# Gadersd/stable-diffusion-burn

Hardware: NVIDIA H100
Metric: images_per_sec_512x512_20steps (higher is better)
Workload: dtype fp16 tensor-core operands (3-term split-fp16 on the two high-res UNet levels), fp32 accumulate

## Files before the change

### stable_diffusion_burn_b200/csrc/api.cu

```cuda
#include "../../include/sdb200.h"

#include <dlfcn.h>

#include <cstdlib>
#include <cstring>
#include <mutex>

#include "attention.cuh"
#include "kernels.cuh"
#include "model.cuh"
#include "runtime.cuh"

using namespace sdb;

struct sdb_ctx {
  Ctx c;
};

static thread_local std::string g_err;

#define API_BEGIN(ctxp)                      \
  if (!(ctxp)) {                             \
    g_err = "null context";                  \
    return 1;                                \
// ... 474 lines not shown
    c.opt_splitk_chunk = value < 1 ? 1 : value;
  else if (k == "attn_split")
    c.opt_attn_split = value;
  else if (k == "attn_regsplit")
    g_attn_regsplit = value;
  else if (k == "emb_hoist")
    c.opt_emb_hoist = value;
  else if (k == "prefetch_w")
    c.opt_prefetch_w = value;
  else if (k == "mlp_passes")
    c.opt_mlp_passes = value;
  else if (k == "gn_epilogue")
    c.opt_gn_epilogue = value;
  else if (k == "skip_merge")
    c.opt_skip_merge = value;
  else if (k == "gn_apply_ctas")
    g_gn_apply_ctas = value < 1 ? 1 : value;
  else if (k == "gn_min_pix")
    g_gn_min_pix = value < 1 ? 1 : value;
  else
    throw Error("unknown option: " + k);
  model_invalidate_graphs(c);
  API_END
}

int sdb_profile_enable(sdb_ctx* ctx, int on) {
  API_BEGIN(ctx)
  profile_collect(c);
  c.profiling = on != 0;
  API_END
// ... 406 lines not shown
```

### stable_diffusion_burn_b200/csrc/gemm_tc.cu

```cuda
#include "gemm_tc.cuh"

#include <cstring>

namespace sdb {

static constexpr int BM = 128;
static constexpr int BK = 64;
static constexpr int A_TILE_BYTES = BM * BK * 2;

template <int BN, int PASSES>
struct StageLayout {
  static constexpr int B_TILE_BYTES = BN * BK * 2;
  static constexpr int A_TILES = PASSES >= 2 ? 2 : 1;
  static constexpr int B_TILES = PASSES >= 3 ? 2 : 1;
  static constexpr int BYTES = A_TILES * A_TILE_BYTES + B_TILES * B_TILE_BYTES;
};
template <int BN>
struct AccLayout {
  static constexpr int PITCH = (BN + 4) * 4;
  static constexpr int BYTES = BM * PITCH;
  static constexpr int GN_BYTES = 32 * 1024;
};
static constexpr int EW = 8;

__device__ __noinline__ void epilogue_store(float4 f, unsigned int o32, unsigned int o16, float* out_f32, __half* out_f16,
                                            __half* out_f16_lo, int act) {
  if (act == 1) {
    f.x = __fdividef(f.x, 1.0f + __expf(-1.702f * f.x)), f.y = __fdividef(f.y, 1.0f + __expf(-1.702f * f.y));
    f.z = __fdividef(f.z, 1.0f + __expf(-1.702f * f.z)), f.w = __fdividef(f.w, 1.0f + __expf(-1.702f * f.w));
  }
  if (out_f32) *reinterpret_cast<float4*>(out_f32 + o32) = f;
  if (out_f16) {
    __half2 h[2] = {f2h2_sat(f.x, f.y), f2h2_sat(f.z, f.w)};
    *reinterpret_cast<uint2*>(out_f16 + o16) = *reinterpret_cast<uint2*>(h);
    if (out_f16_lo) {
      const float2 f0 = __half22float2(h[0]), f1 = __half22float2(h[1]);
      __half2 l[2] = {__floats2half2_rn(f.x - f0.x, f.y - f0.y), __floats2half2_rn(f.z - f1.x, f.w - f1.y)};
      *reinterpret_cast<uint2*>(out_f16_lo + o16) = *reinterpret_cast<uint2*>(l);
    }
  }
}

struct GnTile {
  int tn, img0, tile, nimg;
};
__device__ __forceinline__ GnTile gn_tile_of(const GemmParams& p, int n0, int th, int tw) {
  GnTile g;
  if (p.gn_rpi) {
    g.nimg = p.gn_nimg;
    if (p.gn_rpi >= BM)
      g.tn = 1, g.img0 = (tw * BM) / p.gn_rpi, g.tile = ((tw * BM) % p.gn_rpi) / BM;
    else
      g.tn = BM / p.gn_rpi, g.img0 = tw * g.tn, g.tile = 0;
  } else {
    g.tn = p.TN, g.img0 = n0, g.tile = th * p.tiles_w + tw, g.nimg = p.nimg;
  }
  return g;
}
__device__ __forceinline__ void gn_write_partials(const GemmParams& p, const float2* cs, int BN, int te, int nthreads, const GnTile g,
                                                  int col0, int z) {
// ... 8 lines not shown
      const float2* src = cs + q * BN + b * p.gn_bucket;
      for (int c = 0; c < p.gn_bucket; ++c) sm += src[c].x, sq += src[c].y;
    }
    if (qpi >= 2) sm += __shfl_xor_sync(0xffffffffu, sm, 1), sq += __shfl_xor_sync(0xffffffffu, sq, 1);
    if (qpi == 4) sm += __shfl_xor_sync(0xffffffffu, sm, 2), sq += __shfl_xor_sync(0xffffffffu, sq, 2);
    const int k = q / qpi, img = g.img0 + k, c0 = b * p.gn_bucket;
    if (b < nbk_tile && (q % qpi) == 0 && img < g.nimg && col0 + c0 < p.N) {
      float2* dst = reinterpret_cast<float2*>(p.gn_part) + ((size_t)img * p.gn_cap + slot) * nbk_total + (col0 + c0) / p.gn_bucket;
      *dst = make_float2(sm, sq);
    }
  }
}

enum : int { EPI_PLAIN = 0, EPI_GN = 1, EPI_LNS = 2, EPI_LNC = 3, EPI_GEGLU = 4, EPI_GEGLU_LNC = 5 };

template <int BN, int PASSES, int STAGES>
__host__ __device__ constexpr int region_bytes() {
  return STAGES * StageLayout<BN, PASSES>::BYTES > AccLayout<BN>::BYTES + AccLayout<BN>::GN_BYTES
             ? STAGES * StageLayout<BN, PASSES>::BYTES
             : AccLayout<BN>::BYTES + AccLayout<BN>::GN_BYTES;
}

template <int BN, int PASSES, int STAGES, int EPI>
__global__ void __launch_bounds__(128 + 32 * EW, 1)
gemm_tc_kernel(const __grid_constant__ GemmMaps maps, const GemmParams p) {
  constexpr bool kGN = EPI == EPI_GN, kLNS = EPI == EPI_LNS, kLNC = EPI == EPI_LNC || EPI == EPI_GEGLU_LNC;
  constexpr bool kGEGLU = EPI == EPI_GEGLU || EPI == EPI_GEGLU_LNC;
  using L = StageLayout<BN, PASSES>;
  constexpr int EG = EW / 4;
  constexpr int CSTEP = 32 * EG;
  extern __shared__ __align__(1024) uint8_t smem_raw[];
  uint8_t* smem = smem_raw + ((1024u - (smem_u32(smem_raw) & 1023u)) & 1023u);
  uint64_t* full_bar = reinterpret_cast<uint64_t*>(smem + region_bytes<BN, PASSES, STAGES>());
  uint64_t* empty_bar = full_bar + STAGES;

  const int warp = threadIdx.x >> 5;
  const int lane = threadIdx.x & 31;
  long long* const dbg = (p.dbg && blockIdx.x == 0 && blockIdx.y == 0 && blockIdx.z == 0) ? p.dbg : nullptr;
  if (dbg && threadIdx.x == 0) dbg[0] = clock64();
  if (!p.pdl_late) pdl_trigger();

  int mt = blockIdx.x;
  const int tw = mt % p.tiles_w;
  mt /= p.tiles_w;
  const int th = mt % p.tiles_h;
  const int tn = mt / p.tiles_h;
  const int w0 = tw * p.TW, h0 = th * p.TH, n0 = tn * p.TN;
  const int col0 = blockIdx.y * BN;
// ... 69 lines not shown
      for (int it = it_begin + npre; it < it_end; ++it) {
        mbar_wait(&empty_bar[s], ph ^ 1);
        mbar_expect_tx(&full_bar[s], L::BYTES);
        load_a(it, s);
        load_b(it, s);
        if (++s == STAGES) {
          s = 0;
          ph ^= 1;
        }
      }
    }
  } else if (warp >= 4) {
    pdl_wait();
    const int wg = (warp - 4) >> 2;
    {
      float acc[BN / 2];
#pragma unroll
      for (int i = 0; i < BN / 2; ++i) acc[i] = 0.f;
      int s = 0, prev = -1;
      uint32_t ph = 0;
      for (int it = it_begin; it < it_end; ++it) {
        mbar_wait(&full_bar[s], ph);
        if (dbg && threadIdx.x == 128 && it == it_begin) dbg[3] = clock64();
        const uint32_t a_hi = smem_u32(smem + s * L::BYTES) + wg * (64 * 128);
        const uint32_t a_lo = a_hi + A_TILE_BYTES;
        const uint32_t b_hi = smem_u32(smem + s * L::BYTES) + L::A_TILES * A_TILE_BYTES;
        const uint32_t b_lo = b_hi + L::B_TILE_BYTES;
        wgmma_fence();
#pragma unroll
        for (int k = 0; k < BK / 16; ++k) {
          const uint32_t koff = k * 32;
          const uint64_t da = make_sdesc_sw128(a_hi + koff);
          const uint64_t db = make_sdesc_sw128(b_hi + koff);
          Wgmma<BN>::template ss<0>(acc, da, db, 1);
          if (PASSES >= 2) Wgmma<BN>::template ss<0>(acc, make_sdesc_sw128(a_lo + koff), db, 1);
          if (PASSES >= 3) Wgmma<BN>::template ss<0>(acc, da, make_sdesc_sw128(b_lo + koff), 1);
        }
        wgmma_commit();
        wgmma_wait<1>();
        if (prev >= 0 && lane == 0) mbar_arrive(&empty_bar[prev]);
        prev = s;
        if (++s == STAGES) {
          s = 0;
          ph ^= 1;
        }
      }
      wgmma_wait<0>();
      reg_fence(acc);
      if (dbg && threadIdx.x == 128) dbg[4] = clock64();
      asm volatile("bar.sync 1, %0;" ::"n"(EW * 32) : "memory");
      float* img = reinterpret_cast<float*>(smem);
      const int r0 = wg * 64 + (warp & 3) * 16 + (lane >> 2);
#pragma unroll
      for (int j = 0; j < BN / 2; j += 2) {
        const int row = r0 + 8 * ((j >> 1) & 1), col = 8 * (j >> 2) + 2 * (lane & 3);
        *reinterpret_cast<float2*>(img + row * (AccLayout<BN>::PITCH / 4) + col) = make_float2(acc[j], acc[j + 1]);
      }
      asm volatile("bar.sync 1, %0;" ::"n"(EW * 32) : "memory");
    }
    const int q = warp & 3;
    const int half = (warp - 4) >> 2;
    const int r = q * 32 + lane;
    const int pw = w0 + r % p.TW;
    const int phh = h0 + (r / p.TW) % p.TH;
    const int pn = n0 + r / (p.TW * p.TH);
    const int row_ok = ((pw < p.W) && (phh < p.H) && (pn < p.nimg)) ? 1 : 0;
    const int m = row_ok ? ((pn * p.OH + phh * p.os + p.oa + up_a) * p.OW + pw * p.os + p.ob + up_b) : -1;

    const int sub = lane >> 3;
    const int cq = (lane & 7) * 4;
    constexpr int NCHUNK = (BN + CSTEP - 1) / CSTEP;
    int mr8[8], ao[8];
    float4 bvs[NCHUNK], ad[8];
    const float* ad_ptr = p.residual ? p.residual : p.rowbias;
    const bool res_pair = p.res_hi != nullptr;
    const bool plain = p.split_k == 1 && !kGEGLU;
    float ln_mu = 0.f, ln_rs = 0.f;
    float mu8[8], rs8[8];
    float4 us[NCHUNK];
    if constexpr (kLNC) {
      if (m >= 0) {
        const float2* sp = reinterpret_cast<const float2*>(p.ln_in) + (size_t)m * p.ln_in_slots;
        float sm = 0.f, sq = 0.f;
        for (int i = 0; i < p.ln_in_slots; ++i) {
          const float2 v = sp[i];
          sm += v.x, sq += v.y;
        }
        const float inv = 1.0f / (float)p.ln_C;
        ln_mu = sm * inv;
        ln_rs = rsqrtf(fmaxf(sq * inv - ln_mu * ln_mu, 0.f) + p.ln_eps);
      }
    }
    {
      const bool use_res = p.residual != nullptr;
#pragma unroll
      for (int i = 0; i < 8; ++i) {
        const int rr = i * 4 + sub;
        const int mr = __shfl_sync(0xffffffffu, m, rr);
        const int pnr = __shfl_sync(0xffffffffu, pn, rr);
        mr8[i] = mr;
        ao[i] = res_pair ? mr * p.ldc16 : (use_res ? mr * p.ldc : pnr * p.N);
        ad[i] = make_float4(0.f, 0.f, 0.f, 0.f);
        if constexpr (kLNC) mu8[i] = __shfl_sync(0xffffffffu, ln_mu, rr), rs8[i] = __shfl_sync(0xffffffffu, ln_rs, rr);
      }
      if constexpr (kLNC) {
#pragma unroll
        for (int j = 0; j < NCHUNK; ++j) {
          const int col = col0 + half * 32 + j * CSTEP + cq;
          us[j] = make_float4(0.f, 0.f, 0.f, 0.f);
          if (half * 32 + j * CSTEP < BN && col < p.N) us[j] = *reinterpret_cast<const float4*>(p.ln_u + col);
        }
      }
#pragma unroll
      for (int j = 0; j < NCHUNK; ++j) {
        const int col = col0 + half * 32 + j * CSTEP + cq;
        bvs[j] = make_float4(0.f, 0.f, 0.f, 0.f);
        if (plain && p.bias && half * 32 + j * CSTEP < BN && col < p.N) bvs[j] = *reinterpret_cast<const float4*>(p.bias + col);
      }
    }
    auto issue_addends = [&](int col) {
      if constexpr (kLNC) return;
      if (col >= p.N) return;
      if (res_pair) {
#pragma unroll
        for (int i = 0; i < 8; ++i)
          if (mr8[i] >= 0) {
            const uint2 h = *reinterpret_cast<const uint2*>(p.res_hi + (unsigned)(ao[i] + col));
            const uint2 l = *reinterpret_cast<const uint2*>(p.res_lo + (unsigned)(ao[i] + col));
            const float2 h0 = __half22float2(*reinterpret_cast<const __half2*>(&h.x)), h1 = __half22float2(*reinterpret_cast<const __half2*>(&h.y));
            const float2 l0 = __half22float2(*reinterpret_cast<const __half2*>(&l.x)), l1 = __half22float2(*reinterpret_cast<const __half2*>(&l.y));
            ad[i] = make_float4(h0.x + l0.x, h0.y + l0.y, h1.x + l1.x, h1.y + l1.y);
          }
        return;
      }
      if (ad_ptr == nullptr) return;
#pragma unroll
      for (int i = 0; i < 8; ++i)
        if (mr8[i] >= 0) ad[i] = *reinterpret_cast<const float4*>(ad_ptr + (unsigned)(ao[i] + col));
    };
    const bool pre_issued = plain;
    if (pre_issued) issue_addends(col0 + half * 32 + cq);

    if (p.pdl_late) pdl_trigger();
    if (dbg && threadIdx.x == 128) dbg[5] = clock64();
    constexpr uint32_t TROW = AccLayout<BN>::PITCH;
    const uint32_t arow = smem_u32(smem) + q * 32 * TROW;
    auto unstage = [&](uint32_t t, int rr) {
      float4 f;
      asm volatile("ld.shared.v4.f32 {%0, %1, %2, %3}, [%4];"
                   : "=f"(f.x), "=f"(f.y), "=f"(f.z), "=f"(f.w)
                   : "r"(t + rr * TROW + cq * 4)
                   : "memory");
      return f;
    };
    float2* const gn_cs = reinterpret_cast<float2*>(smem + AccLayout<BN>::BYTES);
    const GnTile gnt = gn_tile_of(p, n0, th, tw);
    auto store_out = [&](float4 f, int mr, int col) {
      epilogue_store(f, (unsigned)(mr * p.ldc + col), (unsigned)(mr * p.ldc16 + col), p.out_f32, p.out_f16, p.out_f16_lo, p.act);
    };

    if (!kGEGLU && p.split_k > 1) {
      const size_t Mtot = (size_t)p.nimg * p.OH * p.OW;
      float* wsbase = p.ws + (size_t)kz * Mtot * p.N;
#pragma unroll 1
      for (int c = half * 32; c < BN; c += CSTEP) {
        const int col = col0 + c + cq;
#pragma unroll
        for (int i = 0; i < 8; ++i) {
          const int rr = i * 4 + sub;
          const int mr = __shfl_sync(0xffffffffu, m, rr);
          if (mr >= 0 && col < p.N) __stcg(reinterpret_cast<float4*>(wsbase + (size_t)mr * p.N + col), unstage(arow + c * 4, rr));
        }
      }
      __threadfence();
      asm volatile("bar.sync 1, %0;" ::"n"(EW * 32) : "memory");
      unsigned int* tk = p.tickets + 2 * ((size_t)blockIdx.y * gridDim.x + blockIdx.x);
// ... 3 lines not shown
        while (atomicAdd(tk, 0u) < (unsigned)p.split_k) {
          __nanosleep(32);
          if (clock64() - t0 > 4000000000ll) __trap();
        }
        __threadfence();
      }
      asm volatile("bar.sync 1, %0;" ::"n"(EW * 32) : "memory");
      {
        const int rows_per = (BM + p.split_k - 1) / p.split_k;
        const int r0 = kz * rows_per, r1 = min(BM, r0 + rows_per);
        constexpr int C4 = BN / 4;
        constexpr int RL = (EW * 32) / C4;
        const int te = threadIdx.x - 128;
        const int rlane = te / C4, cg4 = te - rlane * C4;
        const int rpi = BM / gnt.tn;
        float4* const gn_red = reinterpret_cast<float4*>(smem + AccLayout<BN>::BYTES);
#pragma unroll 1
        for (int k = 0; k < gnt.tn; ++k) {
        float4 gsum = make_float4(0.f, 0.f, 0.f, 0.f), gsq = gsum;
        const int row_a = max(r0, k * rpi), row_b = min(r1, (k + 1) * rpi);
#pragma unroll 1
        for (int rl = row_a + rlane; rlane < RL && rl < row_b; rl += RL) {
          const int col = col0 + cg4 * 4;
          const int qw = w0 + rl % p.TW, qh = h0 + (rl / p.TW) % p.TH, qn = n0 + rl / (p.TW * p.TH);
          if (qw < p.W && qh < p.H && qn < p.nimg && col < p.N) {
            const int mr = (qn * p.OH + qh * p.os + p.oa) * p.OW + qw * p.os + p.ob;
            float4 bv = make_float4(0.f, 0.f, 0.f, 0.f), rb = bv, rs = bv;
            if (p.bias) bv = *reinterpret_cast<const float4*>(p.bias + col);
            if (p.rowbias) rb = *reinterpret_cast<const float4*>(p.rowbias + (size_t)qn * p.N + col);
            if (p.residual) rs = *reinterpret_cast<const float4*>(p.residual + (size_t)mr * p.ldc + col);
            if (p.res_hi) {
// ... 88 lines not shown
              tx.x = rrs * (tx.x - rmu * ux.x), tx.y = rrs * (tx.y - rmu * ux.y), tx.z = rrs * (tx.z - rmu * ux.z), tx.w = rrs * (tx.w - rmu * ux.w);
              tg.x = rrs * (tg.x - rmu * ug.x), tg.y = rrs * (tg.y - rmu * ug.y), tg.z = rrs * (tg.z - rmu * ug.z), tg.w = rrs * (tg.w - rmu * ug.w);
            }
            float4 y;
            y.x = (tx.x + bx.x) * gelu_erf_fast(tg.x + bg.x);
            y.y = (tx.y + bx.y) * gelu_erf_fast(tg.y + bg.y);
            y.z = (tx.z + bx.z) * gelu_erf_fast(tg.z + bg.z);
            y.w = (tx.w + bx.w) * gelu_erf_fast(tg.w + bg.w);
            epilogue_store(y, 0u, (unsigned)(mr * p.ldc16 + ocol0 + c + cq), nullptr, p.out_f16, p.out_f16_lo, 0);
          }
        }
      }
    } else {
      constexpr int NCH = NCHUNK;
      if (!pre_issued) issue_addends(col0 + half * 32 + cq);
      float lrs[8], lrq[8];
#pragma unroll
      for (int k = 0; k < 8; ++k) lrs[k] = 0.f, lrq[k] = 0.f;
      (void)lrs, (void)lrq;
#pragma unroll
      for (int j = 0; j < NCH; ++j) {
        const int c = half * 32 + j * CSTEP;
        if (c < BN) {
          const int col = col0 + c + cq;
          float4 gsum = make_float4(0.f, 0.f, 0.f, 0.f), gsq = gsum;
          (void)gsum, (void)gsq;
          if (col < p.N) {
            const uint32_t tl = arow + c * 4 + sub * TROW + cq * 4;
#pragma unroll
            for (int b4 = 0; b4 < 2; ++b4) {
              float4 t[4];
#pragma unroll
              for (int i = 0; i < 4; ++i)
                asm volatile("ld.shared.v4.f32 {%0, %1, %2, %3}, [%4];"
                             : "=f"(t[i].x), "=f"(t[i].y), "=f"(t[i].z), "=f"(t[i].w)
                             : "r"(tl + (b4 * 4 + i) * 4 * TROW)
                             : "memory");
#pragma unroll
              for (int i = 0; i < 4; ++i) {
                const int k = b4 * 4 + i;
                if (mr8[k] < 0) continue;
                float4 f = t[i];
                if constexpr (kLNC) {
                  f.x = rs8[k] * (f.x - mu8[k] * us[j].x), f.y = rs8[k] * (f.y - mu8[k] * us[j].y);
                  f.z = rs8[k] * (f.z - mu8[k] * us[j].z), f.w = rs8[k] * (f.w - mu8[k] * us[j].w);
// ... 22 lines not shown
              gsum.z += __shfl_xor_sync(0xffffffffu, gsum.z, o), gsum.w += __shfl_xor_sync(0xffffffffu, gsum.w, o);
              gsq.x += __shfl_xor_sync(0xffffffffu, gsq.x, o), gsq.y += __shfl_xor_sync(0xffffffffu, gsq.y, o);
              gsq.z += __shfl_xor_sync(0xffffffffu, gsq.z, o), gsq.w += __shfl_xor_sync(0xffffffffu, gsq.w, o);
            }
            if (sub == 0) {
              float2* d = gn_cs + q * BN + c + cq;
              d[0] = make_float2(gsum.x, gsq.x), d[1] = make_float2(gsum.y, gsq.y);
              d[2] = make_float2(gsum.z, gsq.z), d[3] = make_float2(gsum.w, gsq.w);
            }
          }
          if (j + 1 < NCH && c + CSTEP < BN) issue_addends(col0 + c + CSTEP + cq);
        }
      }
      if constexpr (kLNS) {
#pragma unroll
        for (int k = 0; k < 8; ++k) {
#pragma unroll
          for (int o = 1; o <= 4; o <<= 1) {
            lrs[k] += __shfl_xor_sync(0xffffffffu, lrs[k], o);
            lrq[k] += __shfl_xor_sync(0xffffffffu, lrq[k], o);
          }
        }
        if ((lane & 7) == 0) {
          const int slot = blockIdx.y * 2 + half;
#pragma unroll
          for (int k = 0; k < 8; ++k)
            if (mr8[k] >= 0) {
              float2* d = reinterpret_cast<float2*>(p.ln_out) + (size_t)mr8[k] * p.ln_slots + slot;
              d[0] = make_float2(lrs[k], lrq[k]);
              if (EG == 1) d[1] = make_float2(0.f, 0.f);
            }
        }
      }
      if constexpr (kGN) {
        asm volatile("bar.sync 1, %0;" ::"n"(EW * 32) : "memory");
        gn_write_partials(p, gn_cs, BN, threadIdx.x - 128, EW * 32, gnt, col0, p.up2 ? (int)blockIdx.z * p.gn_phase_slots : 0);
      }
    }
    if (dbg && threadIdx.x == 128) dbg[6] = clock64();
  }
  __syncthreads();
  if (dbg && threadIdx.x == 0) dbg[7] = clock64();
}

static constexpr int SMEM_OPTIN_MAX = 227 * 1024;
template <int BN, int PASSES>
constexpr int pick_stages() {
  constexpr int per = StageLayout<BN, PASSES>::BYTES;
  constexpr int n = (SMEM_OPTIN_MAX - 1024) / (per + 2 * 8);
  return n > 8 ? 8 : n;
}

template <int BN, int PASSES, int STAGES, int EPI>
static void launch_epi(const GemmMaps& maps, const GemmParams& p, cudaStream_t stream) {
  constexpr int smem = region_bytes<BN, PASSES, STAGES>() + 2 * STAGES * 8 + 1024;
  static_assert(smem <= SMEM_OPTIN_MAX, "shared memory per block");
  static_assert(4 * BN * 8 <= AccLayout<BN>::GN_BYTES && 2 * (EW * 32) * 4 * 16 <= AccLayout<BN>::GN_BYTES,
                "GroupNorm column sums must fit in the scratch after the accumulator image");
  static DeviceOnce once;
  if (once.first())
    SDB_CUDA(cudaFuncSetAttribute(gemm_tc_kernel<BN, PASSES, STAGES, EPI>, cudaFuncAttributeMaxDynamicSharedMemorySize, smem));
  dim3 grid(p.tiles_n * p.tiles_h * p.tiles_w, (p.N + BN - 1) / BN, p.up2 ? 4 : p.split_k);
  launch_k(gemm_tc_kernel<BN, PASSES, STAGES, EPI>, grid, dim3(128 + 32 * EW), (size_t)smem, stream, maps, p);
}
template <int BN, int PASSES, int STAGES>
static void launch_inst(const GemmMaps& maps, const GemmParams& p, cudaStream_t stream) {
  SDB_CHECK((p.gn_part != nullptr) + (p.ln_out != nullptr) + (p.ln_in != nullptr) <= 1, "one statistics role per launch");
  if constexpr (BN == 128) {
    if (p.geglu) {
      SDB_CHECK(!p.gn_part && !p.ln_out && p.split_k == 1, "GEGLU epilogue: no statistics output, no split-K");
      return p.ln_in ? launch_epi<BN, PASSES, STAGES, EPI_GEGLU_LNC>(maps, p, stream)
                     : launch_epi<BN, PASSES, STAGES, EPI_GEGLU>(maps, p, stream);
    }
  }
  SDB_CHECK(!p.geglu, "the GEGLU epilogue is built for 128-wide tiles");
  if constexpr (BN >= 128) {
    if (p.gn_part) return launch_epi<BN, PASSES, STAGES, EPI_GN>(maps, p, stream);
  }
  if constexpr (BN == 160) {
    if (p.ln_out) return launch_epi<BN, PASSES, STAGES, EPI_LNS>(maps, p, stream);
  }
  if constexpr (BN == 128 || BN == 160) {
    if (p.ln_in) return launch_epi<BN, PASSES, STAGES, EPI_LNC>(maps, p, stream);
  }
  SDB_CHECK(!p.gn_part && !p.ln_out && !p.ln_in, "this statistics epilogue is not built for this tile width");
  launch_epi<BN, PASSES, STAGES, EPI_PLAIN>(maps, p, stream);
}
bool gemm_tc_supports(int BN, int epi) {
  return epi == EPI_PLAIN || (epi == EPI_GN && BN >= 128) || (epi == EPI_LNS && BN == 160) || (epi == EPI_LNC && (BN == 128 || BN == 160));
}

template <int BN, int PASSES>
static void launch_bn(const GemmMaps& maps, const GemmParams& p, cudaStream_t stream) {
  launch_inst<BN, PASSES, pick_stages<BN, PASSES>()>(maps, p, stream);
}

void gemm_tc_launch(const GemmMaps& maps, const GemmParams& p, int BN, int passes, cudaStream_t stream) {
  SDB_CHECK(p.TN * p.TH * p.TW == BM, "M tile must cover 128 rows");
  SDB_CHECK(p.N % 32 == 0, "N must be a multiple of 32");
#define SDB_DISPATCH(bn)                                             \
  case bn:                                                           \
    if (passes == 1) launch_bn<bn, 1>(maps, p, stream);              \
    else if (passes == 2) launch_bn<bn, 2>(maps, p, stream);         \
    else launch_bn<bn, 3>(maps, p, stream);                          \
    break;
  switch (BN) {
    SDB_DISPATCH(64)
    SDB_DISPATCH(128)
    SDB_DISPATCH(160)
    SDB_DISPATCH(256)
    default:
      throw Error("unsupported BN");
  }
#undef SDB_DISPATCH
}

}
```

### stable_diffusion_burn_b200/csrc/gemm_tc.cuh

```cuda
#pragma once
#include "common.cuh"

namespace sdb {

struct GemmMaps {
  CUtensorMap a[4][2];
  CUtensorMap bx[2];
  CUtensorMap b[2];
};

struct GemmParams {
  int nimg, H, W;
  int TN, TH, TW;
  int tiles_n, tiles_h, tiles_w;
  int N;
  int kc;
  int kc0;
  int num_taps;
  int xkc, xkc0;
  int8_t tap_dh[9], tap_dw[9], tap_ph[9];
  int split_k;
  int up2, gn_phase_slots;
  float* out_f32;
  __half* out_f16;
// ... 16 lines not shown
  const float* ln_in;
  int ln_in_slots, ln_C;
  float ln_eps;
  const float* ln_u;
  const __half* res_hi;
  const __half* res_lo;
  float* ws;
  unsigned int* tickets;
  int OH, OW, os, oa, ob;
};

struct GemmLaunch {
  int BN, passes, stages;
};

void gemm_tc_launch(const GemmMaps& maps, const GemmParams& p, int BN, int passes, cudaStream_t stream);
bool gemm_tc_supports(int BN, int epi);
int gemm_tc_smem_bytes(int BN, int passes, int stages);

}
```

### stable_diffusion_burn_b200/csrc/runtime.cu

```cuda
#include "runtime.cuh"

#include <algorithm>

#include <cudaTypedefs.h>

#include <cmath>
#include <cstdlib>
#include <cstring>

namespace sdb {

int g_pdl_late = 1;
bool g_pdl_enabled = true;
int g_num_sms = 132;

void Arena::init(size_t bytes) {
  SDB_CUDA(cudaMalloc(&base, bytes));
  cap = bytes;
  off = 0;
}
void Arena::destroy() {
  if (base) cudaFree(base);
  base = nullptr;
  cap = off = 0;
// ... 193 lines not shown
    for (int jj = 0; jj < 4; ++jj)
      fprintf(stderr, "  j=%d softmax warpgroup 0: s_issued %lld s_ready %lld softmax_done %lld pv_issued %lld pv_done %lld\n",
              8 + jj, rel(jj * 8 + 0), rel(jj * 8 + 1), rel(jj * 8 + 2), rel(jj * 8 + 3), rel(jj * 8 + 4));
  }
}

static int pow2_floor(int x) {
  int p = 1;
  while (p * 2 <= x) p *= 2;
  return p;
}
static int pow2_ceil(int x) {
  int p = 1;
  while (p < x) p *= 2;
  return p;
}

void run_gemm(Ctx& c, int kind, const ActOp& a0in, const ActOp* a1in, const WeightOp& w, int passes, const Epilogue& ep,
              const ExtraK* xk) {
  ActOp a0 = a0in, a1;
  if (a1in) a1 = *a1in;
  int gn_rpi = ep.gn_rpi, gn_nimg = 0;
  const int kind_in = kind;
  if (kind == G_CONV1) {
    gn_rpi = a0.H * a0.W;
    a0.W = a0.n * a0.H * a0.W, a0.H = 1, a0.n = 1;
    if (a1in) a1.W = a1.n * a1.H * a1.W, a1.H = 1, a1.n = 1;
    kind = G_LINEAR;
  }
  SDB_CHECK(a0.C % 64 == 0, "A channels must be a multiple of 64");
// ... 47 lines not shown
    default:
      throw Error("bad gemm kind");
  }
  SDB_CHECK(w.K == p.num_taps * Ctot, "weight K does not match the operand");
  if (xk) {
    const int xC = xk->x0.C + (xk->has_x1 ? xk->x1.C : 0);
    SDB_CHECK(kind == G_CONV3 || kind == G_LINEAR, "extra-K operands need an unshifted output grid");
    SDB_CHECK(xk->x0.n == a0.n && xk->x0.H == a0.H && xk->x0.W == a0.W && xk->x0.P == 1 && xk->x0.C % 64 == 0, "extra-K geometry");
    SDB_CHECK(!xk->has_x1 || (xk->x1.n == a0.n && xk->x1.H == a0.H && xk->x1.W == a0.W && xk->x1.C % 64 == 0), "extra-K geometry");
    SDB_CHECK(xk->w.N == w.N && xk->w.K == xC, "extra-K weights");
    SDB_CHECK(passes < 2 || (xk->x0.p.lo && (!xk->has_x1 || xk->x1.p.lo)), "multi-pass GEMM needs the lo half of the extra operands");
    SDB_CHECK(passes < 3 || xk->w.p.lo, "3-pass GEMM needs the lo half of the extra weights");
    p.xkc0 = xk->x0.C / 64, p.xkc = xC / 64;
  }

  p.TW = std::min(pow2_floor(a0.W), 128);
  p.TH = std::min(128 / p.TW, pow2_ceil(a0.H));
  p.TN = 128 / (p.TW * p.TH);
  p.tiles_w = (a0.W + p.TW - 1) / p.TW;
  p.tiles_h = (a0.H + p.TH - 1) / p.TH;
  p.tiles_n = (a0.n + p.TN - 1) / p.TN;
  const int m_tiles = p.tiles_w * p.tiles_h * p.tiles_n;

  int BN;
  if (ep.geglu)
    BN = 128;
  else if (w.N % 160 == 0)
    BN = 160;
  else if (w.N % 256 == 0 && (long long)m_tiles * (w.N / 256) >= 2 * g_num_sms)
    BN = 256;
  else if (w.N % 128 == 0)
    BN = 128;
  else
    BN = 64;
  if (ep.ln_out) {
    SDB_CHECK(w.N % 160 == 0 && !ep.geglu, "LayerNorm statistics need an output width that tiles by 160");
    BN = 160;
// ... 4 lines not shown

  const int iters = p.num_taps * p.kc + p.xkc;
  int split = 1;
  if (c.opt_splitk && kind != G_CONV3_UP2 && !ep.geglu && !ep.ln_out && !ep.ln_in) {
    const int ctas = m_tiles * n_tiles;
    if (ctas <= g_num_sms / 2 && iters >= c.opt_splitk_min_iters) {
      split = std::min(std::min(g_num_sms / ctas, iters / c.opt_splitk_chunk), 16);
      if (split < 1) split = 1;
    }
  }
  if (split > 1) {
    const int per = (iters + split - 1) / split;
    split = (iters + per - 1) / per;
  }
  p.split_k = split;
  static const bool gemm_dbg = getenv("SDB_GEMM_DBG") != nullptr || getenv("SDB_LABEL_LOG") != nullptr;
  if (c.debug_sync || c.profiling || gemm_dbg) {
    char buf[256];
    snprintf(buf, sizeof(buf), "gemm kind=%d n=%d H=%d W=%d P=%d C0=%d C1=%d N=%d K=%d xk=%d BN=%d split=%d passes=%d geglu=%d epi=%s%s tile=%dx%dx%d",
             kind, a0.n, a0.H, a0.W, a0.P, a0.C, a1in ? a1.C : 0, w.N, w.K, p.xkc * 64, BN, split, passes, ep.geglu,
             ep.gn ? "gn" : (ep.ln_out ? "lns" : (ep.ln_in ? "lnc" : "-")), ep.residual16.hi ? "+r16" : (ep.residual ? "+r32" : ""), p.TN, p.TH, p.TW);
    c.dbg_label = buf;
  }

  GnPart* gn = ep.gn;
  if (gn) {
    int slots = m_tiles / p.tiles_n * split * phases_out;
    bool geom = p.TN <= 4;
    if (kind == G_LINEAR && gn_rpi > 0) {
      const long long rows = (long long)a0.W;
// ... 22 lines not shown
  p.ln_u = passes >= 3 ? ep.ln_u_full : ep.ln_u_hi;
  SDB_CHECK(!ep.ln_in || (p.ln_u && ep.ln_in_slots > 0 && ep.ln_C == w.K && kind == G_LINEAR), "LayerNorm-consuming GEMM: arguments");
  SDB_CHECK(!ep.ln_in || (!ep.residual && !ep.rowbias && !ep.residual16.hi), "LayerNorm-consuming GEMM: no residual / row bias");
  SDB_CHECK(!ep.ln_out || kind == G_LINEAR, "LayerNorm statistics: rows must be tokens");
  p.res_hi = ep.residual16.hi, p.res_lo = ep.residual16.lo;
  SDB_CHECK(!ep.residual16.hi || (ep.residual16.lo && !ep.residual && !ep.rowbias), "fp16-pair residual: needs both halves, excludes the fp32 residual / row bias");
  p.out_f32 = ep.out_f32;
  p.out_f16 = ep.out_f16.hi;
  p.out_f16_lo = ep.out_f16.lo;
  p.bias = ep.bias;
  p.rowbias = ep.rowbias;
  p.residual = ep.residual;
  p.geglu = ep.geglu;
  p.act = ep.act;
  p.pdl_late = g_pdl_late;
  p.prefetch_w = (g_pdl_enabled && c.opt_prefetch_w && m_tiles <= 4) ? 1 : 0;
  const int nout = ep.geglu ? w.N / 2 : w.N;
  p.ldc = ep.ldc ? ep.ldc : nout;
  p.ldc16 = ep.ldc16 ? ep.ldc16 : nout;
  SDB_CHECK(!(ep.rowbias && ep.residual), "epilogue takes a time-embedding row or a residual, not both");
  p.os = (kind == G_CONV3_UP2) ? 2 : 1;
  p.OH = a0.H * p.os, p.OW = a0.W * p.os;
  SDB_CHECK((double)a0.n * p.OH * p.OW * (double)std::max(p.ldc, p.ldc16) < 2147483648.0,
            "GEMM output exceeds 2^31 elements (the epilogue uses 32-bit element offsets)");

  GemmMaps maps;
  memset(&maps, 0, sizeof(maps));
  maps.a[0][0] = make_act_map(a0.p.hi, a0.C, a0.W, a0.H, a0.P, a0.n, p.TW, p.TH, p.TN);
  maps.a[0][1] = maps.a[0][0];
  if (passes >= 2) maps.a[0][1] = make_act_map(a0.p.lo, a0.C, a0.W, a0.H, a0.P, a0.n, p.TW, p.TH, p.TN);
  maps.a[1][0] = maps.a[0][0];
// ... 50 lines not shown
      SDB_CHECK((long long)m_tiles * n_tiles * split <= g_num_sms, "split-K CTAs must be co-resident");
      p.tickets = c.splitk_tickets;
    }
    {
      static const bool dbg_on = getenv("SDB_GEMM_DBG") != nullptr;
      static long long* dbg_buf = nullptr;
      if (dbg_on) {
        if (!dbg_buf) SDB_CUDA(cudaMallocManaged(&dbg_buf, 16 * sizeof(long long)));
        SDB_CUDA(cudaStreamSynchronize(c.stream));
        memset(dbg_buf, 0, 16 * sizeof(long long));
        p.dbg = dbg_buf;
      }
      const std::string label = c.dbg_label;
      {
        KernelScope ks(c, KC_GEMM, flops * phases_out, bytes * phases_out, flops * passes * phases_out);
        gemm_tc_launch(maps, p, BN, passes, c.stream);
      }
      if (dbg_on) {
        SDB_CUDA(cudaStreamSynchronize(c.stream));
        fprintf(stderr, "gemm_dbg %s | cycles since entry: prologue %lld tma0 %lld landed %lld lastmma %lld accum %lld epi %lld exit %lld | chunk0: ld %lld stage %lld finish %lld (bias %lld loads0 %lld batch0 %lld)\n",
                label.c_str(), dbg_buf[1] - dbg_buf[0], dbg_buf[2] - dbg_buf[0], dbg_buf[3] - dbg_buf[0],
                dbg_buf[4] - dbg_buf[0], dbg_buf[5] - dbg_buf[0], dbg_buf[6] - dbg_buf[0], dbg_buf[7] - dbg_buf[0], dbg_buf[9] - dbg_buf[8], dbg_buf[10] - dbg_buf[9],
                dbg_buf[11] - dbg_buf[10], dbg_buf[12] - dbg_buf[10], dbg_buf[13] - dbg_buf[12], dbg_buf[14] - dbg_buf[13]);
      }
    }
  }
}

}
```

### stable_diffusion_burn_b200/csrc/runtime.cuh

```cuda
#pragma once
#include <string>
#include <unordered_map>
#include <unordered_set>
#include <vector>

#include "common.cuh"
#include "attention.cuh"
#include "gemm_tc.cuh"
#include "kernels.cuh"

namespace sdb {

struct Arena {
  char* base = nullptr;
  size_t cap = 0, off = 0, high = 0;
  void init(size_t bytes);
  void destroy();
  void* alloc(size_t bytes);
  template <class T>
  T* get(size_t count) {
    return reinterpret_cast<T*>(alloc(count * sizeof(T)));
  }
  void reset() { off = 0; }
};
// ... 91 lines not shown
  bool finalized = false;
  std::vector<MetaCheck> meta;
  std::unordered_set<std::string> group_norms;
  std::unordered_map<std::string, float> norm_eps;
  int opt_precision = 0;
  int opt_graphs = 1;
  int opt_splitk = 1;
  int opt_splitk_min_iters = 32, opt_splitk_chunk = 8;
  int opt_skip_merge = 1;
  int opt_raw16 = 1;
  int opt_mlp_passes = 0;
  int opt_attn_split = 1;
  int opt_emb_hoist = 1;
  int opt_prefetch_w = 0;
  int opt_gn_epilogue = 1;
  int sampler_kind = 0;
  double sampler_eta = 0.0;
  uint64_t sampler_noise_seed = 0;
  bool profiling = false;
  std::vector<ProfEvent> prof;
  int64_t launches = 0;
  double cls_ms[KC_COUNT] = {0}, cls_flops[KC_COUNT] = {0}, cls_bytes[KC_COUNT] = {0};
  double cls_issued[KC_COUNT] = {0};
  int64_t cls_launches[KC_COUNT] = {0};
  struct IoBuf {
    void* p = nullptr;
    size_t cap = 0;
  } iobuf[12];
  void* io(int slot, size_t bytes);
  void io_destroy();
// ... 62 lines not shown
```

Baseline: 4.972.

## Add 64-row M tiles for linear GEMMs chosen by a wave-cost model

Templates the wgmma GEMM kernel on BM so linear layers can use 64-row M tiles. In that mode the two consumer warpgroups split the N dimension instead of M, and the epilogue handles fewer rows per warp. A simple wave-quantization cost model picks 64 or 128 rows per linear GEMM when split-K is off and the epilogue is plain or LayerNorm. This is meant to cut tail-wave waste on small-M linears (text encoder, low-res attention projections). In exchange, more CTAs each reuse operands less, and the model's fixed-cost constant is a guess.

```diff
diff --git a/stable_diffusion_burn_b200/csrc/api.cu b/stable_diffusion_burn_b200/csrc/api.cu
--- a/stable_diffusion_burn_b200/csrc/api.cu
+++ b/stable_diffusion_burn_b200/csrc/api.cu
@@ -512,6 +512,10 @@
     c.opt_gn_epilogue = value;
   else if (k == "skip_merge")
     c.opt_skip_merge = value;
+  else if (k == "linear_bm") {
+    SDB_CHECK(value == 0 || value == 64 || value == 128, "linear_bm: 0 (tile plan), 64 or 128");
+    c.opt_linear_bm = value;
+  }
   else if (k == "gn_apply_ctas")
     g_gn_apply_ctas = value < 1 ? 1 : value;
   else if (k == "gn_min_pix")
diff --git a/stable_diffusion_burn_b200/csrc/gemm_tc.cu b/stable_diffusion_burn_b200/csrc/gemm_tc.cu
--- a/stable_diffusion_burn_b200/csrc/gemm_tc.cu
+++ b/stable_diffusion_burn_b200/csrc/gemm_tc.cu
@@ -4,18 +4,17 @@
 
 namespace sdb {
 
-static constexpr int BM = 128;
 static constexpr int BK = 64;
-static constexpr int A_TILE_BYTES = BM * BK * 2;
-
-template <int BN, int PASSES>
+
+template <int BM, int BN, int PASSES>
 struct StageLayout {
+  static constexpr int A_TILE_BYTES = BM * BK * 2;
   static constexpr int B_TILE_BYTES = BN * BK * 2;
   static constexpr int A_TILES = PASSES >= 2 ? 2 : 1;
   static constexpr int B_TILES = PASSES >= 3 ? 2 : 1;
   static constexpr int BYTES = A_TILES * A_TILE_BYTES + B_TILES * B_TILE_BYTES;
 };
-template <int BN>
+template <int BM, int BN>
 struct AccLayout {
   static constexpr int PITCH = (BN + 4) * 4;
   static constexpr int BYTES = BM * PITCH;
@@ -44,6 +43,7 @@
 struct GnTile {
   int tn, img0, tile, nimg;
 };
+template <int BM>
 __device__ __forceinline__ GnTile gn_tile_of(const GemmParams& p, int n0, int th, int tw) {
   GnTile g;
   if (p.gn_rpi) {
@@ -82,24 +82,29 @@
 
 enum : int { EPI_PLAIN = 0, EPI_GN = 1, EPI_LNS = 2, EPI_LNC = 3, EPI_GEGLU = 4, EPI_GEGLU_LNC = 5 };
 
-template <int BN, int PASSES, int STAGES>
+template <int BM, int BN, int PASSES, int STAGES>
 __host__ __device__ constexpr int region_bytes() {
-  return STAGES * StageLayout<BN, PASSES>::BYTES > AccLayout<BN>::BYTES + AccLayout<BN>::GN_BYTES
-             ? STAGES * StageLayout<BN, PASSES>::BYTES
-             : AccLayout<BN>::BYTES + AccLayout<BN>::GN_BYTES;
-}
-
-template <int BN, int PASSES, int STAGES, int EPI>
+  return STAGES * StageLayout<BM, BN, PASSES>::BYTES > AccLayout<BM, BN>::BYTES + AccLayout<BM, BN>::GN_BYTES
+             ? STAGES * StageLayout<BM, BN, PASSES>::BYTES
+             : AccLayout<BM, BN>::BYTES + AccLayout<BM, BN>::GN_BYTES;
+}
+
+template <int BM, int BN, int PASSES, int STAGES, int EPI>
 __global__ void __launch_bounds__(128 + 32 * EW, 1)
 gemm_tc_kernel(const __grid_constant__ GemmMaps maps, const GemmParams p) {
   constexpr bool kGN = EPI == EPI_GN, kLNS = EPI == EPI_LNS, kLNC = EPI == EPI_LNC || EPI == EPI_GEGLU_LNC;
   constexpr bool kGEGLU = EPI == EPI_GEGLU || EPI == EPI_GEGLU_LNC;
-  using L = StageLayout<BN, PASSES>;
+  static_assert(BM == 128 || (BM == 64 && !kGN && !kGEGLU && BN % 16 == 0), "64-row tiles: plain / LayerNorm epilogues");
+  using L = StageLayout<BM, BN, PASSES>;
+  constexpr int A_TILE_BYTES = L::A_TILE_BYTES;
+  constexpr int WN = BM == 128 ? BN : BN / 2;
+  constexpr int RW = BM / 4;
+  constexpr int NR = RW / 4;
   constexpr int EG = EW / 4;
   constexpr int CSTEP = 32 * EG;
   extern __shared__ __align__(1024) uint8_t smem_raw[];
   uint8_t* smem = smem_raw + ((1024u - (smem_u32(smem_raw) & 1023u)) & 1023u);
-  uint64_t* full_bar = reinterpret_cast<uint64_t*>(smem + region_bytes<BN, PASSES, STAGES>());
+  uint64_t* full_bar = reinterpret_cast<uint64_t*>(smem + region_bytes<BM, BN, PASSES, STAGES>());
   uint64_t* empty_bar = full_bar + STAGES;
 
   const int warp = threadIdx.x >> 5;
@@ -199,17 +204,17 @@
     pdl_wait();
     const int wg = (warp - 4) >> 2;
     {
-      float acc[BN / 2];
-#pragma unroll
-      for (int i = 0; i < BN / 2; ++i) acc[i] = 0.f;
+      float acc[WN / 2];
+#pragma unroll
+      for (int i = 0; i < WN / 2; ++i) acc[i] = 0.f;
       int s = 0, prev = -1;
       uint32_t ph = 0;
       for (int it = it_begin; it < it_end; ++it) {
         mbar_wait(&full_bar[s], ph);
         if (dbg && threadIdx.x == 128 && it == it_begin) dbg[3] = clock64();
-        const uint32_t a_hi = smem_u32(smem + s * L::BYTES) + wg * (64 * 128);
+        const uint32_t a_hi = smem_u32(smem + s * L::BYTES) + (BM == 128 ? wg * (64 * 128) : 0);
         const uint32_t a_lo = a_hi + A_TILE_BYTES;
-        const uint32_t b_hi = smem_u32(smem + s * L::BYTES) + L::A_TILES * A_TILE_BYTES;
+        const uint32_t b_hi = smem_u32(smem + s * L::BYTES) + L::A_TILES * A_TILE_BYTES + (BM == 128 ? 0 : wg * (WN * 128));
         const uint32_t b_lo = b_hi + L::B_TILE_BYTES;
         wgmma_fence();
 #pragma unroll
@@ -217,9 +222,9 @@
           const uint32_t koff = k * 32;
           const uint64_t da = make_sdesc_sw128(a_hi + koff);
           const uint64_t db = make_sdesc_sw128(b_hi + koff);
-          Wgmma<BN>::template ss<0>(acc, da, db, 1);
-          if (PASSES >= 2) Wgmma<BN>::template ss<0>(acc, make_sdesc_sw128(a_lo + koff), db, 1);
-          if (PASSES >= 3) Wgmma<BN>::template ss<0>(acc, da, make_sdesc_sw128(b_lo + koff), 1);
+          Wgmma<WN>::template ss<0>(acc, da, db, 1);
+          if (PASSES >= 2) Wgmma<WN>::template ss<0>(acc, make_sdesc_sw128(a_lo + koff), db, 1);
+          if (PASSES >= 3) Wgmma<WN>::template ss<0>(acc, da, make_sdesc_sw128(b_lo + koff), 1);
         }
         wgmma_commit();
         wgmma_wait<1>();
@@ -235,33 +240,34 @@
       if (dbg && threadIdx.x == 128) dbg[4] = clock64();
       asm volatile("bar.sync 1, %0;" ::"n"(EW * 32) : "memory");
       float* img = reinterpret_cast<float*>(smem);
-      const int r0 = wg * 64 + (warp & 3) * 16 + (lane >> 2);
-#pragma unroll
-      for (int j = 0; j < BN / 2; j += 2) {
-        const int row = r0 + 8 * ((j >> 1) & 1), col = 8 * (j >> 2) + 2 * (lane & 3);
-        *reinterpret_cast<float2*>(img + row * (AccLayout<BN>::PITCH / 4) + col) = make_float2(acc[j], acc[j + 1]);
+      const int r0 = (BM == 128 ? wg * 64 : 0) + (warp & 3) * 16 + (lane >> 2);
+      const int c0 = BM == 128 ? 0 : wg * WN;
+#pragma unroll
+      for (int j = 0; j < WN / 2; j += 2) {
+        const int row = r0 + 8 * ((j >> 1) & 1), col = c0 + 8 * (j >> 2) + 2 * (lane & 3);
+        *reinterpret_cast<float2*>(img + row * (AccLayout<BM, BN>::PITCH / 4) + col) = make_float2(acc[j], acc[j + 1]);
       }
       asm volatile("bar.sync 1, %0;" ::"n"(EW * 32) : "memory");
     }
     const int q = warp & 3;
     const int half = (warp - 4) >> 2;
-    const int r = q * 32 + lane;
+    const int r = q * RW + lane;
     const int pw = w0 + r % p.TW;
     const int phh = h0 + (r / p.TW) % p.TH;
     const int pn = n0 + r / (p.TW * p.TH);
-    const int row_ok = ((pw < p.W) && (phh < p.H) && (pn < p.nimg)) ? 1 : 0;
+    const int row_ok = ((lane < RW) && (pw < p.W) && (phh < p.H) && (pn < p.nimg)) ? 1 : 0;
     const int m = row_ok ? ((pn * p.OH + phh * p.os + p.oa + up_a) * p.OW + pw * p.os + p.ob + up_b) : -1;
 
     const int sub = lane >> 3;
     const int cq = (lane & 7) * 4;
     constexpr int NCHUNK = (BN + CSTEP - 1) / CSTEP;
-    int mr8[8], ao[8];
-    float4 bvs[NCHUNK], ad[8];
+    int mr8[NR], ao[NR];
+    float4 bvs[NCHUNK], ad[NR];
     const float* ad_ptr = p.residual ? p.residual : p.rowbias;
     const bool res_pair = p.res_hi != nullptr;
     const bool plain = p.split_k == 1 && !kGEGLU;
     float ln_mu = 0.f, ln_rs = 0.f;
-    float mu8[8], rs8[8];
+    float mu8[NR], rs8[NR];
     float4 us[NCHUNK];
     if constexpr (kLNC) {
       if (m >= 0) {
@@ -279,7 +285,7 @@
     {
       const bool use_res = p.residual != nullptr;
 #pragma unroll
-      for (int i = 0; i < 8; ++i) {
+      for (int i = 0; i < NR; ++i) {
         const int rr = i * 4 + sub;
         const int mr = __shfl_sync(0xffffffffu, m, rr);
         const int pnr = __shfl_sync(0xffffffffu, pn, rr);
@@ -308,7 +314,7 @@
       if (col >= p.N) return;
       if (res_pair) {
 #pragma unroll
-        for (int i = 0; i < 8; ++i)
+        for (int i = 0; i < NR; ++i)
           if (mr8[i] >= 0) {
             const uint2 h = *reinterpret_cast<const uint2*>(p.res_hi + (unsigned)(ao[i] + col));
             const uint2 l = *reinterpret_cast<const uint2*>(p.res_lo + (unsigned)(ao[i] + col));
@@ -320,7 +326,7 @@
       }
       if (ad_ptr == nullptr) return;
 #pragma unroll
-      for (int i = 0; i < 8; ++i)
+      for (int i = 0; i < NR; ++i)
         if (mr8[i] >= 0) ad[i] = *reinterpret_cast<const float4*>(ad_ptr + (unsigned)(ao[i] + col));
     };
     const bool pre_issued = plain;
@@ -328,8 +334,8 @@
 
     if (p.pdl_late) pdl_trigger();
     if (dbg && threadIdx.x == 128) dbg[5] = clock64();
-    constexpr uint32_t TROW = AccLayout<BN>::PITCH;
-    const uint32_t arow = smem_u32(smem) + q * 32 * TROW;
+    constexpr uint32_t TROW = AccLayout<BM, BN>::PITCH;
+    const uint32_t arow = smem_u32(smem) + q * RW * TROW;
     auto unstage = [&](uint32_t t, int rr) {
       float4 f;
       asm volatile("ld.shared.v4.f32 {%0, %1, %2, %3}, [%4];"
@@ -338,13 +344,13 @@
                    : "memory");
       return f;
     };
-    float2* const gn_cs = reinterpret_cast<float2*>(smem + AccLayout<BN>::BYTES);
-    const GnTile gnt = gn_tile_of(p, n0, th, tw);
+    float2* const gn_cs = reinterpret_cast<float2*>(smem + AccLayout<BM, BN>::BYTES);
+    const GnTile gnt = gn_tile_of<BM>(p, n0, th, tw);
     auto store_out = [&](float4 f, int mr, int col) {
       epilogue_store(f, (unsigned)(mr * p.ldc + col), (unsigned)(mr * p.ldc16 + col), p.out_f32, p.out_f16, p.out_f16_lo, p.act);
     };
 
-    if (!kGEGLU && p.split_k > 1) {
+    if (BM == 128 && !kGEGLU && p.split_k > 1) {
       const size_t Mtot = (size_t)p.nimg * p.OH * p.OW;
       float* wsbase = p.ws + (size_t)kz * Mtot * p.N;
 #pragma unroll 1
@@ -378,7 +384,7 @@
         const int te = threadIdx.x - 128;
         const int rlane = te / C4, cg4 = te - rlane * C4;
         const int rpi = BM / gnt.tn;
-        float4* const gn_red = reinterpret_cast<float4*>(smem + AccLayout<BN>::BYTES);
+        float4* const gn_red = reinterpret_cast<float4*>(smem + AccLayout<BM, BN>::BYTES);
 #pragma unroll 1
         for (int k = 0; k < gnt.tn; ++k) {
         float4 gsum = make_float4(0.f, 0.f, 0.f, 0.f), gsq = gsum;
@@ -497,9 +503,9 @@
     } else {
       constexpr int NCH = NCHUNK;
       if (!pre_issued) issue_addends(col0 + half * 32 + cq);
-      float lrs[8], lrq[8];
-#pragma unroll
-      for (int k = 0; k < 8; ++k) lrs[k] = 0.f, lrq[k] = 0.f;
+      float lrs[NR], lrq[NR];
+#pragma unroll
+      for (int k = 0; k < NR; ++k) lrs[k] = 0.f, lrq[k] = 0.f;
       (void)lrs, (void)lrq;
 #pragma unroll
       for (int j = 0; j < NCH; ++j) {
@@ -511,7 +517,7 @@
           if (col < p.N) {
             const uint32_t tl = arow + c * 4 + sub * TROW + cq * 4;
 #pragma unroll
-            for (int b4 = 0; b4 < 2; ++b4) {
+            for (int b4 = 0; b4 < NR / 4; ++b4) {
               float4 t[4];
 #pragma unroll
               for (int i = 0; i < 4; ++i)
@@ -564,7 +570,7 @@
       }
       if constexpr (kLNS) {
 #pragma unroll
-        for (int k = 0; k < 8; ++k) {
+        for (int k = 0; k < NR; ++k) {
 #pragma unroll
           for (int o = 1; o <= 4; o <<= 1) {
             lrs[k] += __shfl_xor_sync(0xffffffffu, lrs[k], o);
@@ -574,7 +580,7 @@
         if ((lane & 7) == 0) {
           const int slot = blockIdx.y * 2 + half;
 #pragma unroll
-          for (int k = 0; k < 8; ++k)
+          for (int k = 0; k < NR; ++k)
             if (mr8[k] >= 0) {
               float2* d = reinterpret_cast<float2*>(p.ln_out) + (size_t)mr8[k] * p.ln_slots + slot;
               d[0] = make_float2(lrs[k], lrq[k]);
@@ -594,71 +600,83 @@
 }
 
 static constexpr int SMEM_OPTIN_MAX = 227 * 1024;
-template <int BN, int PASSES>
+template <int BM, int BN, int PASSES>
 constexpr int pick_stages() {
-  constexpr int per = StageLayout<BN, PASSES>::BYTES;
+  constexpr int per = StageLayout<BM, BN, PASSES>::BYTES;
   constexpr int n = (SMEM_OPTIN_MAX - 1024) / (per + 2 * 8);
   return n > 8 ? 8 : n;
 }
 
-template <int BN, int PASSES, int STAGES, int EPI>
+template <int BM, int BN, int PASSES, int STAGES, int EPI>
 static void launch_epi(const GemmMaps& maps, const GemmParams& p, cudaStream_t stream) {
-  constexpr int smem = region_bytes<BN, PASSES, STAGES>() + 2 * STAGES * 8 + 1024;
+  constexpr int smem = region_bytes<BM, BN, PASSES, STAGES>() + 2 * STAGES * 8 + 1024;
   static_assert(smem <= SMEM_OPTIN_MAX, "shared memory per block");
-  static_assert(4 * BN * 8 <= AccLayout<BN>::GN_BYTES && 2 * (EW * 32) * 4 * 16 <= AccLayout<BN>::GN_BYTES,
+  static_assert(4 * BN * 8 <= AccLayout<BM, BN>::GN_BYTES && 2 * (EW * 32) * 4 * 16 <= AccLayout<BM, BN>::GN_BYTES,
                 "GroupNorm column sums must fit in the scratch after the accumulator image");
   static DeviceOnce once;
   if (once.first())
-    SDB_CUDA(cudaFuncSetAttribute(gemm_tc_kernel<BN, PASSES, STAGES, EPI>, cudaFuncAttributeMaxDynamicSharedMemorySize, smem));
+    SDB_CUDA(cudaFuncSetAttribute(gemm_tc_kernel<BM, BN, PASSES, STAGES, EPI>, cudaFuncAttributeMaxDynamicSharedMemorySize, smem));
   dim3 grid(p.tiles_n * p.tiles_h * p.tiles_w, (p.N + BN - 1) / BN, p.up2 ? 4 : p.split_k);
-  launch_k(gemm_tc_kernel<BN, PASSES, STAGES, EPI>, grid, dim3(128 + 32 * EW), (size_t)smem, stream, maps, p);
-}
-template <int BN, int PASSES, int STAGES>
+  launch_k(gemm_tc_kernel<BM, BN, PASSES, STAGES, EPI>, grid, dim3(128 + 32 * EW), (size_t)smem, stream, maps, p);
+}
+template <int BM, int BN, int PASSES, int STAGES>
 static void launch_inst(const GemmMaps& maps, const GemmParams& p, cudaStream_t stream) {
   SDB_CHECK((p.gn_part != nullptr) + (p.ln_out != nullptr) + (p.ln_in != nullptr) <= 1, "one statistics role per launch");
-  if constexpr (BN == 128) {
-    if (p.geglu) {
-      SDB_CHECK(!p.gn_part && !p.ln_out && p.split_k == 1, "GEGLU epilogue: no statistics output, no split-K");
-      return p.ln_in ? launch_epi<BN, PASSES, STAGES, EPI_GEGLU_LNC>(maps, p, stream)
-                     : launch_epi<BN, PASSES, STAGES, EPI_GEGLU>(maps, p, stream);
-    }
-  }
-  SDB_CHECK(!p.geglu, "the GEGLU epilogue is built for 128-wide tiles");
-  if constexpr (BN >= 128) {
-    if (p.gn_part) return launch_epi<BN, PASSES, STAGES, EPI_GN>(maps, p, stream);
+  if constexpr (BM == 128) {
+    if constexpr (BN == 128) {
+      if (p.geglu) {
+        SDB_CHECK(!p.gn_part && !p.ln_out && p.split_k == 1, "GEGLU epilogue: no statistics output, no split-K");
+        return p.ln_in ? launch_epi<BM, BN, PASSES, STAGES, EPI_GEGLU_LNC>(maps, p, stream)
+                       : launch_epi<BM, BN, PASSES, STAGES, EPI_GEGLU>(maps, p, stream);
+      }
+    }
+    SDB_CHECK(!p.geglu, "the GEGLU epilogue is built for 128-wide tiles");
+    if constexpr (BN >= 128) {
+      if (p.gn_part) return launch_epi<BM, BN, PASSES, STAGES, EPI_GN>(maps, p, stream);
+    }
+  } else {
+    SDB_CHECK(!p.geglu && !p.gn_part && p.split_k == 1 && !p.up2, "64-row tiles: no GEGLU, GroupNorm statistics or split-K");
   }
   if constexpr (BN == 160) {
-    if (p.ln_out) return launch_epi<BN, PASSES, STAGES, EPI_LNS>(maps, p, stream);
+    if (p.ln_out) return launch_epi<BM, BN, PASSES, STAGES, EPI_LNS>(maps, p, stream);
   }
   if constexpr (BN == 128 || BN == 160) {
-    if (p.ln_in) return launch_epi<BN, PASSES, STAGES, EPI_LNC>(maps, p, stream);
+    if (p.ln_in) return launch_epi<BM, BN, PASSES, STAGES, EPI_LNC>(maps, p, stream);
   }
   SDB_CHECK(!p.gn_part && !p.ln_out && !p.ln_in, "this statistics epilogue is not built for this tile width");
-  launch_epi<BN, PASSES, STAGES, EPI_PLAIN>(maps, p, stream);
+  launch_epi<BM, BN, PASSES, STAGES, EPI_PLAIN>(maps, p, stream);
 }
 bool gemm_tc_supports(int BN, int epi) {
   return epi == EPI_PLAIN || (epi == EPI_GN && BN >= 128) || (epi == EPI_LNS && BN == 160) || (epi == EPI_LNC && (BN == 128 || BN == 160));
 }
 
-template <int BN, int PASSES>
+template <int BM, int BN, int PASSES>
 static void launch_bn(const GemmMaps& maps, const GemmParams& p, cudaStream_t stream) {
-  launch_inst<BN, PASSES, pick_stages<BN, PASSES>()>(maps, p, stream);
-}
-
-void gemm_tc_launch(const GemmMaps& maps, const GemmParams& p, int BN, int passes, cudaStream_t stream) {
-  SDB_CHECK(p.TN * p.TH * p.TW == BM, "M tile must cover 128 rows");
+  launch_inst<BM, BN, PASSES, pick_stages<BM, BN, PASSES>()>(maps, p, stream);
+}
+
+void gemm_tc_launch(const GemmMaps& maps, const GemmParams& p, int BM, int BN, int passes, cudaStream_t stream) {
+  SDB_CHECK(BM == 128 || (BM == 64 && (BN == 128 || BN == 160)), "M tile: 128 rows, or 64 rows at BN 128 / 160");
+  SDB_CHECK(p.TN * p.TH * p.TW == BM, "the M tile's TN x TH x TW must cover BM rows");
   SDB_CHECK(p.N % 32 == 0, "N must be a multiple of 32");
-#define SDB_DISPATCH(bn)                                             \
+#define SDB_DISPATCH(bm, bn)                                         \
   case bn:                                                           \
-    if (passes == 1) launch_bn<bn, 1>(maps, p, stream);              \
-    else if (passes == 2) launch_bn<bn, 2>(maps, p, stream);         \
-    else launch_bn<bn, 3>(maps, p, stream);                          \
+    if (passes == 1) launch_bn<bm, bn, 1>(maps, p, stream);          \
+    else if (passes == 2) launch_bn<bm, bn, 2>(maps, p, stream);     \
+    else launch_bn<bm, bn, 3>(maps, p, stream);                      \
     break;
+  if (BM == 64) {
+    switch (BN) {
+      SDB_DISPATCH(64, 128)
+      SDB_DISPATCH(64, 160)
+    }
+    return;
+  }
   switch (BN) {
-    SDB_DISPATCH(64)
-    SDB_DISPATCH(128)
-    SDB_DISPATCH(160)
-    SDB_DISPATCH(256)
+    SDB_DISPATCH(128, 64)
+    SDB_DISPATCH(128, 128)
+    SDB_DISPATCH(128, 160)
+    SDB_DISPATCH(128, 256)
     default:
       throw Error("unsupported BN");
   }
diff --git a/stable_diffusion_burn_b200/csrc/gemm_tc.cuh b/stable_diffusion_burn_b200/csrc/gemm_tc.cuh
--- a/stable_diffusion_burn_b200/csrc/gemm_tc.cuh
+++ b/stable_diffusion_burn_b200/csrc/gemm_tc.cuh
@@ -54,7 +54,7 @@
   int BN, passes, stages;
 };
 
-void gemm_tc_launch(const GemmMaps& maps, const GemmParams& p, int BN, int passes, cudaStream_t stream);
+void gemm_tc_launch(const GemmMaps& maps, const GemmParams& p, int BM, int BN, int passes, cudaStream_t stream);
 bool gemm_tc_supports(int BN, int epi);
 int gemm_tc_smem_bytes(int BN, int passes, int stages);
 
diff --git a/stable_diffusion_burn_b200/csrc/runtime.cu b/stable_diffusion_burn_b200/csrc/runtime.cu
--- a/stable_diffusion_burn_b200/csrc/runtime.cu
+++ b/stable_diffusion_burn_b200/csrc/runtime.cu
@@ -231,6 +231,17 @@
   int p = 1;
   while (p < x) p *= 2;
   return p;
+}
+
+static constexpr double kLinearCtaFixedCycles = 5000.0;
+
+static int linear_tile_rows(int m_tiles128, int m_tiles64, int n_tiles, int BN, int iters, int passes) {
+  auto cost = [&](int bm, int m_tiles) {
+    const long long ctas = (long long)m_tiles * n_tiles;
+    const long long waves = (ctas + g_num_sms - 1) / g_num_sms;
+    return (double)waves * (2.0 * bm * BN * 64.0 * iters * passes / 4096.0 + kLinearCtaFixedCycles);
+  };
+  return cost(64, m_tiles64) < cost(128, m_tiles128) ? 64 : 128;
 }
 
 void run_gemm(Ctx& c, int kind, const ActOp& a0in, const ActOp* a1in, const WeightOp& w, int passes, const Epilogue& ep,
@@ -308,13 +319,16 @@
     p.xkc0 = xk->x0.C / 64, p.xkc = xC / 64;
   }
 
-  p.TW = std::min(pow2_floor(a0.W), 128);
-  p.TH = std::min(128 / p.TW, pow2_ceil(a0.H));
-  p.TN = 128 / (p.TW * p.TH);
-  p.tiles_w = (a0.W + p.TW - 1) / p.TW;
-  p.tiles_h = (a0.H + p.TH - 1) / p.TH;
-  p.tiles_n = (a0.n + p.TN - 1) / p.TN;
-  const int m_tiles = p.tiles_w * p.tiles_h * p.tiles_n;
+  auto set_m_tile = [&](int bm) {
+    p.TW = std::min(pow2_floor(a0.W), bm);
+    p.TH = std::min(bm / p.TW, pow2_ceil(a0.H));
+    p.TN = bm / (p.TW * p.TH);
+    p.tiles_w = (a0.W + p.TW - 1) / p.TW;
+    p.tiles_h = (a0.H + p.TH - 1) / p.TH;
+    p.tiles_n = (a0.n + p.TN - 1) / p.TN;
+    return p.tiles_w * p.tiles_h * p.tiles_n;
+  };
+  int m_tiles = set_m_tile(128);
 
   int BN;
   if (ep.geglu)
@@ -349,6 +363,11 @@
     split = (iters + per - 1) / per;
   }
   p.split_k = split;
+  int BM = 128;
+  if (kind == G_LINEAR && !ep.geglu && !ep.gn && split == 1 && (BN == 128 || BN == 160)) {
+    BM = c.opt_linear_bm ? c.opt_linear_bm : linear_tile_rows(m_tiles, set_m_tile(64), n_tiles, BN, iters, passes);
+    m_tiles = set_m_tile(BM);
+  }
   static const bool gemm_dbg = getenv("SDB_GEMM_DBG") != nullptr || getenv("SDB_LABEL_LOG") != nullptr;
   if (c.debug_sync || c.profiling || gemm_dbg) {
     char buf[256];
@@ -401,7 +420,7 @@
   p.geglu = ep.geglu;
   p.act = ep.act;
   p.pdl_late = g_pdl_late;
-  p.prefetch_w = (g_pdl_enabled && c.opt_prefetch_w && m_tiles <= 4) ? 1 : 0;
+  p.prefetch_w = (g_pdl_enabled && c.opt_prefetch_w && m_tiles * BM <= 4 * 128) ? 1 : 0;
   const int nout = ep.geglu ? w.N / 2 : w.N;
   p.ldc = ep.ldc ? ep.ldc : nout;
   p.ldc16 = ep.ldc16 ? ep.ldc16 : nout;
@@ -482,7 +501,7 @@
       const std::string label = c.dbg_label;
       {
         KernelScope ks(c, KC_GEMM, flops * phases_out, bytes * phases_out, flops * passes * phases_out);
-        gemm_tc_launch(maps, p, BN, passes, c.stream);
+        gemm_tc_launch(maps, p, BM, BN, passes, c.stream);
       }
       if (dbg_on) {
         SDB_CUDA(cudaStreamSynchronize(c.stream));
diff --git a/stable_diffusion_burn_b200/csrc/runtime.cuh b/stable_diffusion_burn_b200/csrc/runtime.cuh
--- a/stable_diffusion_burn_b200/csrc/runtime.cuh
+++ b/stable_diffusion_burn_b200/csrc/runtime.cuh
@@ -129,6 +129,7 @@
   int opt_emb_hoist = 1;
   int opt_prefetch_w = 0;
   int opt_gn_epilogue = 1;
+  int opt_linear_bm = 0;
   int sampler_kind = 0;
   double sampler_eta = 0.0;
   uint64_t sampler_noise_seed = 0;
```

Measured after the change: 5.074 (median of 6 runs). 2.1% higher.
